# theislab/dca

Measured on AMD Instinct MI355X. Metric: cells/sec training (ZINB AE, 68k x 20k), higher is better.
Workload: dtype f32

## Files before the change

### dca_amd/csrc/dcahip_heads.hip

```cpp
#include <hip/hip_runtime.h>
#include <stdint.h>
#include <type_traits>
#include "dcahip.h"
#include "zinb_math.hpp"

namespace {

using f32x16 = __attribute__((ext_vector_type(16))) float;

constexpr int kTG = 32;
constexpr int kTR = 32;
constexpr int kLdS = 33;
constexpr int kWG = 2;
constexpr int kMaxGrid = 2048;
constexpr int kMaxSmallGrid = 8192;
constexpr int kCUs = 256;
constexpr int kZU = 4;
constexpr int kQCap = 320;

__device__ __forceinline__ int rowmap(int e, int hi) { return (e & 3) + 8 * (e >> 2) + 4 * hi; }

__device__ __forceinline__ void wave_sync() {
    __builtin_amdgcn_fence(__ATOMIC_RELEASE, "wavefront");
    __builtin_amdgcn_wave_barrier();
// ... 43 lines not shown
        f[0][j] = a; f[1][j] = b;
    }
}
#ifdef DCA_EXP_H2_TWO
#define MFMA_H3(A, Bf, ACC) { ACC = MFMAH(A[0], Bf[1], ACC); ACC = MFMAH(A[0], Bf[0], ACC); }
#else
#define MFMA_H3(A, Bf, ACC) { ACC = MFMAH(A[1], Bf[0], ACC); ACC = MFMAH(A[0], Bf[1], ACC); ACC = MFMAH(A[0], Bf[0], ACC); }
#endif

__device__ __forceinline__ float pow2i(int e) { return __uint_as_float((unsigned)(127 + e) << 23); }
__device__ __forceinline__ int block_exp(float m) {
    if (!(m > 0.f) || !(m < INFINITY)) return 0;
    const int e = kTop + 1 - __builtin_amdgcn_frexp_expf(m);
    return e < -60 ? -60 : (e > 60 ? 60 : e);
}
__device__ __forceinline__ float wave_max(float v) {
    int l = (int)__builtin_amdgcn_mbcnt_hi(~0u, __builtin_amdgcn_mbcnt_lo(~0u, 0u));
    asm volatile("" : "+v"(l));
#pragma unroll
    for (int off = 32; off > 0; off >>= 1)
        v = fmaxf(v, __int_as_float(__builtin_amdgcn_ds_bpermute((l ^ off) << 2, __float_as_int(v))));
    return v;
}

struct HeadsArgs2 {
    const unsigned short* HA;
    const unsigned short* HT;
    const int* eH;
    const float* H; long ldh;
    float* gW; long ldg;
    float* g_theta;
    const float* Wh; long ldw;
    const float* bh;
    const float* theta_w;
    const float* y;  long ldy;
    const unsigned char* yc; long ldc;
    const int* ovf_ptr; const int* ovf_col; const float* ovf_val;
    const float* sf;
    const int* perm;
    const long long* cursor;
    float* ws_dw;  long dw_stride;
    float* ws_dh;
    int npart, nitems;
    const int* tile_order;
    double* partials;
    long plane, ldws;
    int B, hL, G;
    int S, NT;
    float ridge, inv_n;
    int d_exp;
    int tile_base;
};

__device__ __forceinline__ float escaped_count(const HeadsArgs2& p, long srow, int col) {
    float v = 255.f;
    if (p.ovf_ptr)
        for (int i = p.ovf_ptr[srow], e = p.ovf_ptr[srow + 1]; i < e; ++i)
            if (p.ovf_col[i] == col) { v = p.ovf_val[i]; break; }
    return v;
}

__global__ __launch_bounds__(256) void heads_split_h_kernel(const float* H, long ldh, int B, int hL,
                                                            unsigned short* HA, unsigned short* HT, int* eH) {
    __shared__ unsigned short tr[2][64][32 + 2];
    __shared__ float wm[4];
    const int t = blockIdx.x, tid = threadIdx.x;
    const int row = tid >> 3, k0 = (tid & 7) * 8;
    const long grow = (long)t * 32 + row;
    float x[8];
    float m = 0.f;
#pragma unroll
    for (int j = 0; j < 8; ++j) {
        x[j] = (grow < B && k0 + j < hL) ? H[grow * ldh + k0 + j] : 0.f;
        m = fmaxf(m, fabsf(x[j]));
    }
    m = wave_max(m);
    if ((tid & 63) == 0) wm[tid >> 6] = m;
    __syncthreads();
    const int e = block_exp(fmaxf(fmaxf(wm[0], wm[1]), fmaxf(wm[2], wm[3])));
    if (tid == 0) eH[t] = (fmaxf(fmaxf(wm[0], wm[1]), fmaxf(wm[2], wm[3])) > 0.f) ? e : kEHZero;
    const float sc = pow2i(e);
#pragma unroll
    for (int j = 0; j < 8; ++j) x[j] *= sc;
    u32x4 f[2];
    split8(x, f);
    const int pos = (row & 0x13) | ((row & 4) << 1) | ((row & 8) >> 1);
#pragma unroll
    for (int q = 0; q < 2; ++q) {
        *reinterpret_cast<u32x4*>(HA + (((long)t * 2 + q) * 32 + row) * 64 + k0) = f[q];
#pragma unroll
        for (int j = 0; j < 8; ++j) tr[q][k0 + j][pos] = (unsigned short)(f[q][j >> 1] >> (16 * (j & 1)));
    }
    __syncthreads();
    for (int c = tid; c < 2 * 64 * 4; c += 256) {
        const int q = c >> 8, i = (c >> 2) & 63, part = c & 3;
        u32x4 v;
#pragma unroll
        for (int j = 0; j < 4; ++j) v[j] = (unsigned)tr[q][i][part * 8 + 2 * j] | ((unsigned)tr[q][i][part * 8 + 2 * j + 1] << 16);
        *reinterpret_cast<u32x4*>(HT + (((long)t * 2 + q) * 64 + i) * 32 + part * 8) = v;
    }
}

template <bool HAS_PI, bool CONST_DISP, bool YC>
__global__ __launch_bounds__(64 * kWR2) void heads_fused_h2_kernel(HeadsArgs2 p) {
    using YV = std::conditional_t<YC, unsigned, float>;
    constexpr int WR = kWR2;
    constexpr int NH = 1 + (CONST_DISP ? 0 : 1) + (HAS_PI ? 1 : 0);
    constexpr int PI_H = NH - 1;
    constexpr int KT = 64;
    constexpr int ST_PLANE = kTG * kLdS;
    constexpr int QCAP = 192;
    constexpr int CELL_LD = 144;
    constexpr int HEAD_B = kTG * CELL_LD;
    constexpr int ROWT = 96;
    constexpr int PW_FLOATS = NH * HEAD_B / 4 + (CONST_DISP ? ST_PLANE : 0) + QCAP * 4 + ROWT;
    constexpr int NTHREADS = 64 * WR;
    constexpr int W_PIECE = 64 * 64;
    constexpr int W_FLOATS = NH * 2 * W_PIECE / 4;
    constexpr int NRED = NH * 2 * 16 + NH + 1;
    constexpr int BIAS_FLOATS = (NH + 1) * 32;
    constexpr int LDS_FLOATS = W_FLOATS + WR * PW_FLOATS + BIAS_FLOATS;
    static_assert((WR / 2) * NRED * 64 <= LDS_FLOATS, "dW reduce scratch");
    __shared__ __attribute__((aligned(16))) float lds[LDS_FLOATS];
    __shared__ double lred[WR];
    __shared__ float wmaxs[WR];

    const int tid = threadIdx.x, lane = tid & 63;
    const int wave = __builtin_amdgcn_readfirstlane(tid >> 6);
    const int l31 = lane & 31, hi = lane >> 5;
    const int r = wave;
    const long long cur = p.cursor ? *p.cursor : 0;
    double dacc = 0.0;
    bool first_item = true;
    const int s_wg = blockIdx.x % p.S, wq = blockIdx.x / p.S;
    const int ngb = p.nitems / p.S;
    const int full = ngb / p.npart, rem = ngb - full * p.npart;
    const int nrounds = full + ((rem > 0 && ((full & 1) ? p.npart - 1 - wq : wq) < rem) ? 1 : 0);
    const int kD0 = kDExp0 + p.d_exp;
    int eHmin = 1 << 20;
    for (int t = s_wg * WR + r; t < p.NT; t += p.S * WR) { const int e = p.eH[t]; eHmin = (e != kEHZero && e < eHmin) ? e : eHmin; }
    eHmin = __builtin_amdgcn_readfirstlane(eHmin == (1 << 20) ? 0 : eHmin);
    int srow_l = 0;
    float sf_l = 1.f;
    int eHt = 0;
    u32x4 ha0[2] = {};
    bool carried = false;
#pragma unroll 1
    for (int j = 0; j < nrounds; ++j) {
    const int gb = j * p.npart + ((j & 1) ? p.npart - 1 - wq : wq);
    int s_opaque = s_wg;
    asm volatile("" : "+v"(s_opaque));
    const int s = __builtin_amdgcn_readfirstlane(s_opaque);
    const int gt = p.tile_order ? p.tile_order[gb + p.tile_base] : gb + p.tile_base;
    const int g0 = gt * kTG;
    const int gene = g0 + l31;
    const bool tile_ok = g0 < p.G;
    const bool gvalid = gene < p.G;

    unsigned char* const Wimg = reinterpret_cast<unsigned char*>(lds);
    unsigned char* const Pimg = reinterpret_cast<unsigned char*>(lds + W_FLOATS + wave * PW_FLOATS);
    float* const Th = lds + W_FLOATS + wave * PW_FLOATS + NH * HEAD_B / 4;
    u32x4* const Qe = reinterpret_cast<u32x4*>(lds + W_FLOATS + wave * PW_FLOATS + NH * HEAD_B / 4 + (CONST_DISP ? ST_PLANE : 0));
    float* const Bs = lds + W_FLOATS + WR * PW_FLOATS;
    int* const Rt = reinterpret_cast<int*>(lds + W_FLOATS + wave * PW_FLOATS + PW_FLOATS - ROWT);
    float* const Sft = reinterpret_cast<float*>(Rt + 64);

    const int gene_c = gvalid ? gene : p.G - 1;
    const float* const ycol = p.y + gene_c;
    const unsigned char* const ycolc = p.yc + gene_c;
    const unsigned ldy_u = YC ? (unsigned)p.ldc : (unsigned)p.ldy;
    auto count_at = [&](int sr) -> YV {
        if constexpr (YC) return (unsigned)ycolc[(unsigned long long)(unsigned)sr * ldy_u];
        else return ycol[(unsigned long long)(unsigned)sr * ldy_u];
    };
    YV yA[kZU], yB[kZU];
    auto row_clamped = [&](int tt) { const int rl = tt * kTR + l31; return rl < p.B ? rl : p.B - 1; };
    auto load_srow = [&](int tt) { const int rlc = row_clamped(tt); return p.perm ? p.perm[cur + rlc] : (int)(cur + rlc); };
    const __amdgpu_buffer_rsrc_t ha_rs = __builtin_amdgcn_make_buffer_rsrc(
        const_cast<unsigned short*>(p.HA), 0, p.NT * (kHTile * 2), 0x00020000);
    const int ha_lane = l31 * 128 + hi * 64;
    auto load_ha = [&](int tt, int ks, u32x4 (&dst)[2]) {
        const int so = tt * (kHTile * 2);
        int ha_o = ha_lane;
        asm volatile("" : "+v"(ha_o));
#pragma unroll
        for (int q = 0; q < 2; ++q)
            dst[q] = __builtin_bit_cast(u32x4, __builtin_amdgcn_raw_buffer_load_b128(ha_rs, ha_o + q * 4096 + ks * 16, so, 0));
    };
    const int t0 = s * WR + r;
    if (tile_ok && t0 < p.NT && !carried) {
        srow_l = load_srow(t0);
        eHt = p.eH[t0];
        sf_l = p.sf[srow_l];
        load_ha(t0, 0, ha0);
    }
    auto item_head = [&]() {
        if (lane < 32) Rt[l31] = srow_l;
        wave_sync();
        const int4 r4 = *reinterpret_cast<const int4*>(Rt + 4 * hi);
        yA[0] = count_at(r4.x); yA[1] = count_at(r4.y); yA[2] = count_at(r4.z); yA[3] = count_at(r4.w);
    };

    int eW = 0;
    if (tile_ok) {
        constexpr int UNR = (NH * 64 * 8 + NTHREADS - 1) / NTHREADS;
        constexpr int ITEMS = NH * 64 * 8;
        float4 v[UNR];
        int tidp = tid;
        asm volatile("" : "+v"(tidp));
        float m = 0.f;
#pragma unroll
        for (int u = 0; u < UNR; ++u) {
            const int idx = tidp + u * NTHREADS;
            const int c4 = idx & 7, kq = (idx >> 3) & 63, h = (idx >> 9) < NH ? (idx >> 9) : NH - 1;
            const int kc = kq < p.hL ? kq : p.hL - 1;
            long gcol = g0 + c4 * 4;
            if (gcol > p.plane - 4) gcol = p.plane - 4;
            v[u] = *reinterpret_cast<const float4*>(p.Wh + (long)kc * p.ldw + (long)h * p.plane + gcol);
        }
        float bv[NH + 1];
#pragma unroll
        for (int h = 0; h < NH; ++h) bv[h] = p.bh[(long)h * p.plane + gene_c];
        bv[NH] = CONST_DISP ? p.theta_w[gene_c] : 0.f;
        item_head();
#pragma unroll
        for (int u = 0; u < UNR; ++u) {
            const int idx = tidp + u * NTHREADS;
            const int c4 = idx & 7, kq = (idx >> 3) & 63;
            const int gcol = g0 + c4 * 4;
            const bool kv = idx < ITEMS && kq < p.hL && gcol <= p.plane - 4;
            if (!kv || gcol + 0 >= p.G) v[u].x = 0.f;
            if (!kv || gcol + 1 >= p.G) v[u].y = 0.f;
            if (!kv || gcol + 2 >= p.G) v[u].z = 0.f;
            if (!kv || gcol + 3 >= p.G) v[u].w = 0.f;
            m = fmaxf(fmaxf(m, fmaxf(fabsf(v[u].x), fabsf(v[u].y))), fmaxf(fabsf(v[u].z), fabsf(v[u].w)));
        }
        m = wave_max(m);
        if (lane == 0) wmaxs[wave] = m;
        __syncthreads();
        m = fmaxf(fmaxf(fmaxf(wmaxs[0], wmaxs[1]), fmaxf(wmaxs[2], wmaxs[3])), fmaxf(fmaxf(wmaxs[4], wmaxs[5]), fmaxf(wmaxs[6], wmaxs[7])));
        eW = __builtin_amdgcn_readfirstlane(block_exp(m));
        const float wsc = pow2i(eW);
#pragma unroll
        for (int u = 0; u < UNR; ++u) {
            const int idx = tidp + u * NTHREADS;
            if (idx >= ITEMS) continue;
            const int c4 = idx & 7, kq = (idx >> 3) & 63, h = idx >> 9;
            unsigned a0, a1, b0, b1;
            split_pair(v[u].x * wsc, v[u].y * wsc, a0, a1);
            split_pair(v[u].z * wsc, v[u].w * wsc, b0, b1);
            const int off = kq * 64 + ((((c4 >> 1) + (kq >> 2)) & 3) << 4) + ((c4 & 1) << 3);
            *reinterpret_cast<u32x2*>(Wimg + (h * 2 + 0) * W_PIECE + off) = u32x2{a0, b0};
            *reinterpret_cast<u32x2*>(Wimg + (h * 2 + 1) * W_PIECE + off) = u32x2{a1, b1};
        }
        if (tid < 32) {
#pragma unroll
            for (int h = 0; h < NH; ++h) Bs[h * 32 + tid] = gvalid ? bv[h] : 0.f;
            Bs[NH * 32 + tid] = (CONST_DISP && gvalid) ? bv[NH] : 0.f;
        }
    }
    __syncthreads();

    f32x16 dW[NH][2];
#pragma unroll
    for (int h = 0; h < NH; ++h)
#pragma unroll
        for (int ib = 0; ib < 2; ++ib)
#pragma unroll
            for (int e = 0; e < 16; ++e) dW[h][ib][e] = 0.f;
    float bsum[NH];
#pragma unroll
    for (int h = 0; h < NH; ++h) bsum[h] = 0.f;
    float thsum = 0.f;

    if (tile_ok) {
        const int tstep = p.S * WR;
        int t = t0;
        const long dh_tstride = (long)p.npart * (kTR * KT);
        float* const dh_part = p.ws_dh + (long)(blockIdx.x / p.S) * (kTR * KT);
        const int dh_lane = ((((l31 & 0x13) | ((l31 & 4) << 1) | ((l31 & 8) >> 1)) * KT) + 4 * hi) * 4;
        const __amdgpu_buffer_rsrc_t ht_rs = __builtin_amdgcn_make_buffer_rsrc(
            const_cast<unsigned short*>(p.HT), 0, p.NT * (kHTile * 2), 0x00020000);
        const int ht_lane = l31 * 64 + hi * 16;
        auto load_ht = [&](int tt, int ks, u32x4 (&dst)[2][2]) {
            const int so = tt * (kHTile * 2);
            int ht_o = ht_lane;
            asm volatile("" : "+v"(ht_o));
#pragma unroll
            for (int q = 0; q < 2; ++q)
#pragma unroll
                for (int ib = 0; ib < 2; ++ib)
                    dst[q][ib] = __builtin_bit_cast(u32x4, __builtin_amdgcn_raw_buffer_load_b128(
                        ht_rs, ht_o + q * 4096 + ib * 2048 + ks * 32, so, 0));
        };
// ... 346 lines not shown
                            u32x4 bf[2] = {w_dr(h, 0, jb, gs), w_dr(h, 1, jb, gs)};
                            MFMA_H3(bf, af, dHa[jb])
                        }
                    }
#pragma unroll
                for (int jb = 0; jb < 2; ++jb)
#pragma unroll
                    for (int eq = 0; eq < 4; ++eq) {
                        u32x4 v;
#pragma unroll
                        for (int w = 0; w < 4; ++w) v[w] = __float_as_uint(dHa[jb][4 * eq + w] * fu);
                        __builtin_amdgcn_raw_buffer_store_b128(v, dh_rs, dh_o + 128 * jb + 32 * eq, 0, 0);
                    }
            }
            srow_l = srow_n;
            sf_l = sf_n;
            eHt = eHn;
            if (lane < 32) Sft[l31] = sf_n;
            rb ^= 1;
            wave_sync();
        }
        carried = carried || t0 < p.NT;
        {
#pragma unroll
            for (int h = 0; h < NH; ++h)
#pragma unroll
                for (int ib = 0; ib < 2; ++ib)
#pragma unroll
                    for (int e = 0; e < 16; ++e) dW[h][ib][e] = __builtin_amdgcn_ldexpf(dW[h][ib][e], -accE);
        }
    }

    __syncthreads();

    {
        float* red = lds;
#pragma unroll
        for (int step = 1; step < WR; step *= 2) {
            const int slot = r / (2 * step);
            float* rs = red + (long)slot * NRED * 64 + lane;
            if (r % (2 * step) == step) {
                int n = 0;
#pragma unroll
                for (int h = 0; h < NH; ++h)
#pragma unroll
                    for (int ib = 0; ib < 2; ++ib)
#pragma unroll
                        for (int e = 0; e < 16; ++e) rs[(n++) * 64] = dW[h][ib][e];
#pragma unroll
                for (int h = 0; h < NH; ++h) rs[(n++) * 64] = bsum[h];
                rs[(n++) * 64] = thsum;
            }
            __syncthreads();
            if (r % (2 * step) == 0 && r + step < WR) {
                int n = 0;
#pragma unroll
                for (int h = 0; h < NH; ++h)
#pragma unroll
                    for (int ib = 0; ib < 2; ++ib)
#pragma unroll
                        for (int e = 0; e < 16; ++e) dW[h][ib][e] += rs[(n++) * 64];
#pragma unroll
                for (int h = 0; h < NH; ++h) bsum[h] += rs[(n++) * 64];
                thsum += rs[(n++) * 64];
            }
            __syncthreads();
        }
    }
    if (r == 0 && tile_ok) {
        const bool direct = p.S == 1;
        float* out = direct ? p.gW : p.ws_dw + (long)s * p.dw_stride;
        const long ldo = direct ? p.ldg : p.ldws;
        const float fin = direct ? p.inv_n : 1.f;
        const bool cw = gene < p.plane;
#pragma unroll
        for (int h = 0; h < NH; ++h) {
#pragma unroll
            for (int ib = 0; ib < 2; ++ib)
#pragma unroll
                for (int e = 0; e < 16; ++e) {
                    const int i = ib * 32 + rowmap(e, hi);
                    if (cw && i < p.hL) out[(long)i * ldo + (long)h * p.plane + gene] = dW[h][ib][e] * fin;
                }
            const float bv = bsum[h] + __shfl_xor(bsum[h], 32, 64);
            if (cw && hi == 0) out[(long)p.hL * ldo + (long)h * p.plane + gene] = bv * fin;
        }
        if (CONST_DISP) {
            const float tv = thsum + __shfl_xor(thsum, 32, 64);
            if (direct) {
                if (gvalid && hi == 0) {
                    const float e = expf(p.theta_w[gene]);
                    p.g_theta[gene] = (e >= 1e-3f && e <= 1e4f) ? tv * p.inv_n * e : 0.f;
                }
            } else if (cw && hi == 0) {
                out[(long)(p.hL + 1) * ldo + gene] = tv;
            }
        }
    }
    __syncthreads();
    first_item = false;
    }
// ... 131 lines not shown
    if (loss_out && bid == 0) {
        __shared__ double lsum[256];
        double a = 0.0;
        for (int i = threadIdx.x; i < n_partials; i += 256) a += loss_partials[i];
        lsum[threadIdx.x] = a;
        __syncthreads();
        for (int st = 128; st > 0; st >>= 1) {
            if ((int)threadIdx.x < st) lsum[threadIdx.x] += lsum[threadIdx.x + st];
            __syncthreads();
        }
        if (threadIdx.x == 0) {
            float lf = (float)(lsum[0] * loss_scale);
            if (isnan(lf)) lf = INFINITY;
            *loss_out = lf;
        }
    }
}

template <int GL>
__global__ __launch_bounds__(256) void heads_reduce_dh_kernel(ReduceDhArgs q) { reduce_dh_body<GL>(q, blockIdx.x); }

template <int GL>
__global__ __launch_bounds__(256) void heads_reduce_both_kernel(ReduceDhArgs qh, ReduceDwArgs qw, int n_dh) {
    if ((int)blockIdx.x < n_dh) reduce_dh_body<GL>(qh, blockIdx.x);
    else reduce_dw_body(qw, blockIdx.x - n_dh, gridDim.x - n_dh);
}


struct HeadsPlan {
    bool small;
    int HLB, WR, S, NT, ntg, ngb, grid;
    int nitems, npart;
    long ldws, dw_stride, dw_bytes, dh_bytes, hs_bytes;
    int nmain, ntail, S2, grid2, npart2, nitems2;
    long dh2_bytes, dw2_bytes;
};

inline bool al16(const void* p) { return (reinterpret_cast<uintptr_t>(p) & 15) == 0; }

bool make_heads_plan(int B, int hL, int G, long plane, int flags, HeadsPlan* out) {
    if (flags & (DCAHIP_NLL_POISSON | DCAHIP_NLL_MSE)) return false;
    if (B <= 0 || G <= 0 || hL <= 0 || hL > 64 || plane < G || (plane & 3) || plane > ((G + 31) & ~31)) return false;
    if (B > (1 << 22)) return false;
    const bool has_pi = flags & DCAHIP_NLL_HAS_PI, cdisp = flags & DCAHIP_NLL_CONST_DISP;
    const int NH = 1 + (cdisp ? 0 : 1) + (has_pi ? 1 : 0);
    HeadsPlan p;
    p.HLB = 2;
    p.NT = (B + kTR - 1) / kTR;
    p.ntg = (G + kTG - 1) / kTG;
    p.ngb = p.ntg;
    if (p.ngb > kMaxGrid) return false;
    p.small = p.NT < kWr8MinNT;
    static_assert((kWr8MinNT - 1) * kMaxGrid <= kMaxSmallGrid, "loss partials of the four-wave kernel");
    p.WR = p.small ? 1 : kWR2;
    const int smax = (p.NT + p.WR - 1) / p.WR;
    double best = 1e300;
    p.S = 1;
    const double item_cost = 0.75;
    for (int S = 1; S <= smax && (long)S * p.ngb <= kMaxGrid; ++S) {
        const long items = (long)S * p.ngb;
        const long rounds = (items + kCUs - 1) / kCUs;
        const int tiles = (p.NT + S * p.WR - 1) / (S * p.WR);
        const double cost = (double)rounds * (tiles + item_cost);
        if (cost < best - 1e-9) { best = cost; p.S = S; }
    }
    p.nitems = p.S * p.ngb;
// ... 10 lines not shown
        p.npart = p.grid / p.S;
    }
    p.nmain = p.ngb; p.ntail = 0; p.S2 = 0; p.grid2 = 0; p.npart2 = 0; p.nitems2 = 0;
    if (!p.small && p.S >= 2) {
        const int full = p.ngb / p.npart, rem = p.ngb - full * p.npart;
        const int tiles = (p.NT + p.S * p.WR - 1) / (p.S * p.WR);
        if (full >= 1 && rem > 0) {
            const double uniform = (double)(full + 1) * (tiles + item_cost);
            double best2 = 1e300; int bestS = 0;
            for (int S2 = 2 * p.S; S2 <= smax && (long)S2 * rem <= kMaxGrid; S2 *= 2) {
                const long items2 = (long)S2 * rem;
                const long rounds2 = (items2 + kCUs - 1) / kCUs;
                const int tiles2 = (p.NT + S2 * p.WR - 1) / (S2 * p.WR);
                const double c2 = (double)rounds2 * (tiles2 + item_cost);
                if (c2 < best2 - 1e-9) { best2 = c2; bestS = S2; }
            }
            if (bestS && (double)full * (tiles + item_cost) + best2 + 1.0 < uniform - 0.5) {
                p.nmain = full * p.npart; p.ntail = rem; p.S2 = bestS;
                p.nitems = p.S * p.nmain;
                p.nitems2 = p.S2 * p.ntail;
                const int res2 = kCUs / p.S2 * p.S2;
                p.grid2 = p.nitems2 < res2 ? p.nitems2 : res2;
                p.npart2 = p.grid2 / p.S2;
            }
        }
    }
    p.ldws = (long)NH * plane;
    p.dw_stride = (long)(hL + 2) * p.ldws;
    p.dw_bytes = (long)p.S * p.dw_stride * (long)sizeof(float);
    p.dh_bytes = (long)p.npart * p.NT * kTR * (p.HLB * 32) * (long)sizeof(float);
    p.dw2_bytes = (long)p.S2 * p.dw_stride * (long)sizeof(float);
    p.dh2_bytes = (long)p.npart2 * p.NT * kTR * (p.HLB * 32) * (long)sizeof(float);
    p.hs_bytes = 2L * p.NT * kHTile * 2 + (((long)p.NT * 4 + 15) & ~15L);
    *out = p;
    return true;
}

template <bool HAS_PI, bool CONST_DISP, bool YC>
__global__ __launch_bounds__(256) void heads_fused_small_kernel(HeadsArgs2 p) {
    using YV = std::conditional_t<YC, unsigned, float>;
    constexpr int NH = 1 + (CONST_DISP ? 0 : 1) + (HAS_PI ? 1 : 0);
    constexpr int PI_H = NH - 1;
    constexpr int KT = 64;
    constexpr int ST_PLANE = kTG * kLdS;
    constexpr int NP = NH + (CONST_DISP ? 1 : 0);
    constexpr int TH_P = NH;
    constexpr int ST_TILE = NP * ST_PLANE;
    constexpr int W_PIECE = 64 * 64;
    constexpr int W_FLOATS = NH * 2 * W_PIECE / 4;
    constexpr int BIAS_FLOATS = CONST_DISP ? (NH + 1) * 32 : 0;
    constexpr int NW = 4;
    static_assert(NW * kZU == 16, "one Z group per wave");
    constexpr int QCAP = kZU * 64;
    constexpr int LDS_FLOATS = W_FLOATS + ST_TILE + NW * QCAP + BIAS_FLOATS;
    static_assert(LDS_FLOATS * 4 + NW * 8 + 64 <= 42 * 1280, "three workgroups per CU (LDS is allocated in 1280-byte granules)");
    __shared__ __attribute__((aligned(16))) float lds[LDS_FLOATS];
    __shared__ double lred[NW];
    __shared__ float wmaxs[NW];
    __shared__ float dmaxs[NW];

    const int tid = threadIdx.x, lane = tid & 63;
    const int wave = __builtin_amdgcn_readfirstlane(tid >> 6);
    const int l31 = lane & 31, hi = lane >> 5;
    const long long cur = p.cursor ? *p.cursor : 0;
    const int t = p.NT > 1 ? (int)(blockIdx.x % p.NT) : 0;
    const int gb = p.NT > 1 ? (int)(blockIdx.x / p.NT) : (int)blockIdx.x;
// ... 383 lines not shown
    for (int k0 = 0; k0 < K; k0 += 16) {
        float av[8], bv[8];
#pragma unroll
        for (int j = 0; j < 8; ++j) {
            av[j] = A[(long)l31 * K + k0 + 8 * hi + j] * sa;
            bv[j] = B[(long)(k0 + 8 * hi + j) * 32 + l31] * sb;
        }
        u32x4 af[2], bf[2];
        split8(av, af);
        split8(bv, bf);
        MFMA_H3(af, bf, acc)
    }
    const float un = pow2i(-(ea + eb));
#pragma unroll
    for (int e = 0; e < 16; ++e) C[rowmap(e, hi) * 32 + l31] = acc[e] * un;
}

template <bool P, bool C, bool YC>
void launch_fused(const HeadsPlan& pl, const HeadsArgs2& a, hipStream_t s) {
    if (pl.small) hipLaunchKernelGGL((heads_fused_small_kernel<P, C, YC>), dim3(pl.grid), dim3(256), 0, s, a);
    else hipLaunchKernelGGL((heads_fused_h2_kernel<P, C, YC>), dim3(pl.grid), dim3(64 * kWR2), 0, s, a);
}

}

extern "C" long dcahip_heads_fused_workspace_bytes(int B, int hL, int G, long plane, int flags) {
    HeadsPlan p;
    if (!make_heads_plan(B, hL, G, plane, flags, &p)) return 0;
    long need = 0;
    for (int nt = 1; nt <= p.NT; ++nt) {
        const int b = nt * kTR < B ? nt * kTR : B;
        HeadsPlan q;
        if (!make_heads_plan(b, hL, G, plane, flags, &q)) continue;
        const long n = q.dw_bytes + q.dh_bytes + q.hs_bytes + q.dw2_bytes + q.dh2_bytes;
        if (n > need) need = n;
    }
    return need;
}

extern "C" int dcahip_x3_product_32x32(const float* A, const float* B, float* C, int K, void* stream) {
    if (!A || !B || !C || K <= 0 || (K & 15)) return DCAHIP_EINVAL;
    hipLaunchKernelGGL(x3_product_kernel, dim3(1), dim3(64), 0, static_cast<hipStream_t>(stream), A, B, C, K);
    return (int)hipGetLastError();
}

extern "C" int dcahip_heads_tile_order_len(int G) { return G > 0 ? (((G + kTG - 1) / kTG + kWG - 1) / kWG) * kWG : 0; }

extern "C" int dcahip_heads_fused(const float* H, long ldh, const float* Wh, long ldw,
                                  const float* bh, long plane, const float* theta_w,
                                  const float* y, long ldy,
                                  const unsigned char* yc, long ldc, const int* ovf_ptr, const int* ovf_col,
                                  const float* ovf_val, const float* sf, const int* perm,
                                  const long long* cursor, int B, int hL, int G, float ridge,
                                  float inv_n, int flags, float* gW, long ldg, float* g_theta,
                                  float* dH, long lddh, double* loss_partials, int* n_partials_out,
                                  void* workspace, long workspace_bytes, const int* tile_order,
                                  float* loss_out, int d_exp, void* stream) {
    const bool has_pi = flags & DCAHIP_NLL_HAS_PI, cdisp = flags & DCAHIP_NLL_CONST_DISP;
    HeadsPlan pl;
    if (!make_heads_plan(B, hL, G, plane, flags, &pl)) return DCAHIP_EINVAL;
    if (!H || !Wh || !bh || (!y && !yc) || !sf || !gW || !dH || !loss_partials || !workspace) return DCAHIP_EINVAL;
    if (cdisp && (!theta_w || !g_theta)) return DCAHIP_EINVAL;
    if (workspace_bytes < pl.dw_bytes + pl.dh_bytes + pl.hs_bytes + pl.dw2_bytes + pl.dh2_bytes) return DCAHIP_EINVAL;
    if (!al16(H) || !al16(Wh) || !al16(workspace) || (ldh & 3) || (ldw & 3) || ldh < ((hL + 3) & ~3))
        return DCAHIP_EINVAL;
    if (d_exp > 0 || d_exp < -24 || !(ridge >= 0.f) || ridge > 1e3f) return DCAHIP_EINVAL;
    const int NH = 1 + (cdisp ? 0 : 1) + (has_pi ? 1 : 0);
    if (ldw < (long)NH * plane || ldg < (long)NH * plane) return DCAHIP_EINVAL;
    if (yc ? (ldc < G || ldc > 0xffffffffL) : (ldy < G || ldy > 0xffffffffL)) return DCAHIP_EINVAL;
    float* ws_dh = static_cast<float*>(workspace);
    float* ws_dw = ws_dh + pl.dh_bytes / sizeof(float);
    float* ws_dh2 = ws_dw + pl.dw_bytes / sizeof(float);
    float* ws_dw2 = ws_dh2 + pl.dh2_bytes / sizeof(float);
    hipStream_t s = static_cast<hipStream_t>(stream);
    bool direct_dw = false;
    {
        unsigned short* HA = reinterpret_cast<unsigned short*>(reinterpret_cast<char*>(workspace) + pl.dh_bytes + pl.dw_bytes +
                                                               pl.dh2_bytes + pl.dw2_bytes);
        unsigned short* HT = HA + (long)pl.NT * kHTile;
        int* eH = reinterpret_cast<int*>(HT + (long)pl.NT * kHTile);
        if (!pl.small) {
            hipLaunchKernelGGL(heads_split_h_kernel, dim3(pl.NT), dim3(256), 0, s, H, ldh, B, hL, HA, HT, eH);
            int rc0 = (int)hipGetLastError();
            if (rc0 != 0) return rc0;
        }
        direct_dw = pl.S == 1;
        HeadsArgs2 a{HA, HT, eH, H, ldh, gW, ldg, g_theta, Wh, ldw, bh, theta_w, y, ldy, yc, ldc, ovf_ptr, ovf_col, ovf_val,
                     sf, perm, cursor, ws_dw, pl.dw_stride, ws_dh,
                     pl.npart, pl.nitems, tile_order, loss_partials, plane, pl.ldws, B, hL, G, pl.S, pl.NT, ridge, inv_n, d_exp, 0};
        auto launch = [&](const HeadsPlan& q, const HeadsArgs2& b) {
            if (yc) {
                if (has_pi && cdisp) launch_fused<true, true, true>(q, b, s);
                else if (has_pi) launch_fused<true, false, true>(q, b, s);
                else if (cdisp) launch_fused<false, true, true>(q, b, s);
                else launch_fused<false, false, true>(q, b, s);
            } else {
                if (has_pi && cdisp) launch_fused<true, true, false>(q, b, s);
                else if (has_pi) launch_fused<true, false, false>(q, b, s);
                else if (cdisp) launch_fused<false, true, false>(q, b, s);
                else launch_fused<false, false, false>(q, b, s);
            }
        };
        launch(pl, a);
        if (pl.ntail > 0) {
            HeadsPlan q2 = pl;
            q2.grid = pl.grid2; q2.S = pl.S2;
            HeadsArgs2 b = a;
            b.ws_dw = ws_dw2; b.ws_dh = ws_dh2; b.npart = pl.npart2; b.nitems = pl.nitems2; b.S = pl.S2;
            b.partials = loss_partials + pl.grid; b.tile_base = pl.nmain;
            launch(q2, b);
        }
    }
    int rc = (int)hipGetLastError();
    if (rc != 0) return rc;
    const int n_part = pl.grid + pl.grid2;
    if (n_partials_out) *n_partials_out = n_part;
    {
        const int KT = pl.HLB * 32;
        const long nq = (long)B * (KT / 4);
        const ReduceDhArgs qh{ws_dh, pl.npart, B, pl.NT * kTR, KT, hL, dH, lddh, inv_n, loss_partials, n_part, (double)inv_n, loss_out,
// ... 25 lines not shown
```

### include/dcahip.h

```cpp
#ifndef DCAHIP_H
#define DCAHIP_H

#ifdef __cplusplus
extern "C" {
#endif

#define DCAHIP_VERSION 2
#define DCAHIP_EINVAL (-22)

#define DCAHIP_NLL_HAS_PI      1
#define DCAHIP_NLL_CONST_DISP  2
#define DCAHIP_NLL_POISSON     4
#define DCAHIP_NLL_MSE         8

int dcahip_version(void);

int dcahip_zinb_max_partials(void);

int dcahip_zinb_nll(const float* a_mean, const float* a_disp, const float* a_pi, long lda,
                    const float* theta_w,
                    const float* y, long ldy, const float* sf,
                    const int* perm, const long long* cursor,
                    int B, int G, float ridge, float inv_n, int flags,
                    float* d_mean, float* d_disp, float* d_pi, long ldd,
// ... 20 lines not shown
                         double* cell_out, double* gene_acc, double* workspace, void* stream);

#define DCAHIP_GROUP_NO_SF   16
#define DCAHIP_GROUP_LOG1P   32
int dcahip_group_moments_workspace_doubles(int B, int G, int K);
int dcahip_group_moments(const float* a_mean, long lda, const float* sf, const int* codes,
                         int B, int G, int K, int flags,
                         double* sum_acc, double* sumsq_acc, long ldg,
                         double* workspace, void* stream);

long dcahip_ranksum_workspace_bytes(int g, int n);
int dcahip_ranksum(const float* x, long ldx, int g, int n,
                   const int* order, int m, const int* gstart, int K, int ref,
                   long long* rank2, long long* tie, long ldr,
                   void* workspace, void* stream);

long dcahip_gram_workspace_doubles(int B, int G);
int dcahip_gram(const float* x, long ldx, const int* cols, const int* keep, const double* shift,
                int B, int G, double* cross, long ldc, double* dsum, double* ws, void* stream);

int dcahip_loss_finalize(const double* partials, int n_partials, double scale,
                         float* loss_out, void* stream);

int dcahip_step_end(const float* loss, double weight, float* hist, int rows_per_slot,
                    double* acc, long long* cursor, int advance, void* stream);

int dcahip_zinb_heads_infer(const float* a_mean, const float* a_disp, const float* a_pi,
                            long lda, const float* sf, int B, int G,
                            float* mean_sf, float* theta, float* pi, long ldo, int flags,
                            void* stream);

long dcahip_heads_fused_workspace_bytes(int B, int hL, int G, long plane, int flags);
int dcahip_heads_tile_order_len(int G);
int dcahip_heads_fused(const float* H, long ldh, const float* Wh, long ldw, const float* bh,
                       long plane, const float* theta_w,
                       const float* y, long ldy,
                       const unsigned char* yc, long ldc, const int* ovf_ptr, const int* ovf_col,
                       const float* ovf_val, const float* sf,
                       const int* perm, const long long* cursor,
                       int B, int hL, int G, float ridge, float inv_n, int flags,
                       float* gW, long ldg, float* g_theta, float* dH, long lddh,
                       double* loss_partials, int* n_partials_out,
                       void* workspace, long workspace_bytes, const int* tile_order,
                       float* loss_out, int d_exp, void* stream);
int dcahip_x3_product_32x32(const float* A, const float* B, float* C, int K, void* stream);

int dcahip_sgemm(int ta, int tb, int M, int N, int K,
                 const float* A, long lda, const float* B, long ldb, float* C, long ldc,
                 const float* bias, const int* perm, const long long* cursor,
                 int colsum_row, int split_k, void* workspace, long workspace_bytes,
                 void* stream);
long dcahip_sgemm_workspace_bytes(int ta, int tb, int M, int N, int K, int colsum_row, int split_k);
int dcahip_sgemm_plan(int ta, int tb, int M, int N, int K, int colsum_row, int split_k,
                      const float* A, long lda, const float* B, long ldb, int out[8]);
int dcahip_split_planes(const float* src, long ld, const int* perm, const long long* cursor, long R, int C,
                        void* planes, long ldp, long plane_stride, void* stream);
int dcahip_gemm_p3(int ta, int tb, int M, int N, int K, const void* A, long lda, long plane_a,
                   const void* B, long ldb, long plane_b, float* C, long ldc, const float* bias,
                   const int* perm, const long long* cursor, int colsum_row, int split_k,
                   void* workspace, long workspace_bytes, void* stream);
long dcahip_gemm_p3_workspace_bytes(int M, int N, int K, int colsum_row, int split_k);
int dcahip_gemm_planes_plan(int pieces, int ta, int tb, int M, int N, int K, int gather, int colsum_row, int split_k, int out[12]);
int dcahip_absmax_exp(const float* src, long ld, long R, int C, int* exp_out, void* scratch_word, void* stream);
int dcahip_split_planes_h2(const float* src, long ld, const int* perm, const long long* cursor, long R, int C,
                           void* planes, long ldp, long plane_stride, const int* exp, void* stream);
int dcahip_gemm_h2_supported(int M, int N, int K);
// ... 233 lines not shown
```

Measured before the change: 4.367 million.

## Precompute split weight tile images in split kernel and prefetch next tile during reduce

Moves the per-tile weight split (scaling, bf16-style split into hi/lo pieces, bias/theta gather) out of the fused heads kernel into extra blocks of the H-split kernel, writing a per-tile record to workspace. The fused kernel then just loads the prebuilt record and issues the load for the next tile before the dW reduction, landing it into LDS after, overlapping global latency with reduction. The reduction scratch is shifted past the weight image to avoid clobbering it. It adds workspace memory and a global round-trip for the image.

```diff
diff --git a/dca_amd/csrc/dcahip_heads.hip b/dca_amd/csrc/dcahip_heads.hip
--- a/dca_amd/csrc/dcahip_heads.hip
+++ b/dca_amd/csrc/dcahip_heads.hip
@@ -99,6 +99,7 @@
     float* g_theta;
     const float* Wh; long ldw;
     const float* bh;
+    const unsigned char* wimg;
     const float* theta_w;
     const float* y;  long ldy;
     const unsigned char* yc; long ldc;
@@ -127,11 +128,11 @@
     return v;
 }
 
-__global__ __launch_bounds__(256) void heads_split_h_kernel(const float* H, long ldh, int B, int hL,
-                                                            unsigned short* HA, unsigned short* HT, int* eH) {
+__device__ __forceinline__ void split_h_body(const float* H, long ldh, int B, int hL,
+                                             unsigned short* HA, unsigned short* HT, int* eH, int t) {
     __shared__ unsigned short tr[2][64][32 + 2];
     __shared__ float wm[4];
-    const int t = blockIdx.x, tid = threadIdx.x;
+    const int tid = threadIdx.x;
     const int row = tid >> 3, k0 = (tid & 7) * 8;
     const long grow = (long)t * 32 + row;
     float x[8];
@@ -166,6 +167,79 @@
         for (int j = 0; j < 4; ++j) v[j] = (unsigned)tr[q][i][part * 8 + 2 * j] | ((unsigned)tr[q][i][part * 8 + 2 * j + 1] << 16);
         *reinterpret_cast<u32x4*>(HT + (((long)t * 2 + q) * 64 + i) * 32 + part * 8) = v;
     }
+}
+
+constexpr int kWPiece = 64 * 64;
+constexpr long wimg_rec_bytes(int NH) { return (long)NH * 2 * kWPiece + (NH + 1) * 32 * 4 + 16; }
+struct WImgArgs {
+    const float* Wh; long ldw; const float* bh; const float* theta_w;
+    long plane; int hL, G;
+    unsigned char* out;
+};
+
+template <int NH>
+__device__ __forceinline__ void wimage_body(const WImgArgs& q, int gt) {
+    __shared__ float wmaxs[4];
+    const int tid = threadIdx.x, lane = tid & 63, wave = tid >> 6;
+    const int g0 = gt * kTG;
+    unsigned char* const rec = q.out + (long)gt * wimg_rec_bytes(NH);
+    constexpr int UNR = 2 * NH;
+    float4 v[UNR];
+    float m = 0.f;
+#pragma unroll
+    for (int u = 0; u < UNR; ++u) {
+        const int idx = tid + u * 256;
+        const int c4 = idx & 7, kq = (idx >> 3) & 63, h = idx >> 9;
+        const int kc = kq < q.hL ? kq : q.hL - 1;
+        long gcol = g0 + c4 * 4;
+        if (gcol > q.plane - 4) gcol = q.plane - 4;
+        v[u] = *reinterpret_cast<const float4*>(q.Wh + (long)kc * q.ldw + (long)h * q.plane + gcol);
+    }
+#pragma unroll
+    for (int u = 0; u < UNR; ++u) {
+        const int idx = tid + u * 256;
+        const int c4 = idx & 7, kq = (idx >> 3) & 63;
+        const int gcol = g0 + c4 * 4;
+        const bool kv = kq < q.hL && gcol <= q.plane - 4;
+        if (!kv || gcol + 0 >= q.G) v[u].x = 0.f;
+        if (!kv || gcol + 1 >= q.G) v[u].y = 0.f;
+        if (!kv || gcol + 2 >= q.G) v[u].z = 0.f;
+        if (!kv || gcol + 3 >= q.G) v[u].w = 0.f;
+        m = fmaxf(fmaxf(m, fmaxf(fabsf(v[u].x), fabsf(v[u].y))), fmaxf(fabsf(v[u].z), fabsf(v[u].w)));
+    }
+    m = wave_max(m);
+    if (lane == 0) wmaxs[wave] = m;
+    __syncthreads();
+    const int eW = block_exp(fmaxf(fmaxf(wmaxs[0], wmaxs[1]), fmaxf(wmaxs[2], wmaxs[3])));
+    const float wsc = pow2i(eW);
+#pragma unroll
+    for (int u = 0; u < UNR; ++u) {
+        const int idx = tid + u * 256;
+        const int c4 = idx & 7, kq = (idx >> 3) & 63, h = idx >> 9;
+        unsigned a0, a1, b0, b1;
+        split_pair(v[u].x * wsc, v[u].y * wsc, a0, a1);
+        split_pair(v[u].z * wsc, v[u].w * wsc, b0, b1);
+        const int off = kq * 64 + ((((c4 >> 1) + (kq >> 2)) & 3) << 4) + ((c4 & 1) << 3);
+        *reinterpret_cast<u32x2*>(rec + (h * 2 + 0) * kWPiece + off) = u32x2{a0, b0};
+        *reinterpret_cast<u32x2*>(rec + (h * 2 + 1) * kWPiece + off) = u32x2{a1, b1};
+    }
+    float* const rows = reinterpret_cast<float*>(rec + NH * 2 * kWPiece);
+    if (tid < 32) {
+        const int gene = g0 + tid;
+        const bool gvalid = gene < q.G;
+#pragma unroll
+        for (int h = 0; h < NH; ++h) rows[h * 32 + tid] = gvalid ? q.bh[(long)h * q.plane + gene] : 0.f;
+        rows[NH * 32 + tid] = (q.theta_w && gvalid) ? q.theta_w[gene] : 0.f;
+    } else if (tid < 36) {
+        reinterpret_cast<int*>(rows + (NH + 1) * 32)[tid - 32] = tid == 32 ? eW : 0;
+    }
+}
+
+template <int NH>
+__global__ __launch_bounds__(256) void heads_split_kernel(const float* H, long ldh, int B, int hL, unsigned short* HA,
+                                                          unsigned short* HT, int* eH, int n_h, WImgArgs q) {
+    if ((int)blockIdx.x < n_h) split_h_body(H, ldh, B, hL, HA, HT, eH, blockIdx.x);
+    else wimage_body<NH>(q, blockIdx.x - n_h);
 }
 
 template <bool HAS_PI, bool CONST_DISP, bool YC>
@@ -182,15 +256,17 @@
     constexpr int ROWT = 96;
     constexpr int PW_FLOATS = NH * HEAD_B / 4 + (CONST_DISP ? ST_PLANE : 0) + QCAP * 4 + ROWT;
     constexpr int NTHREADS = 64 * WR;
-    constexpr int W_PIECE = 64 * 64;
+    constexpr int W_PIECE = kWPiece;
     constexpr int W_FLOATS = NH * 2 * W_PIECE / 4;
     constexpr int NRED = NH * 2 * 16 + NH + 1;
-    constexpr int BIAS_FLOATS = (NH + 1) * 32;
+    constexpr int BIAS_FLOATS = (NH + 1) * 32 + 4;
     constexpr int LDS_FLOATS = W_FLOATS + WR * PW_FLOATS + BIAS_FLOATS;
-    static_assert((WR / 2) * NRED * 64 <= LDS_FLOATS, "dW reduce scratch");
+    constexpr int IMG_B = NH * 2 * W_PIECE;
+    constexpr int NBQ = BIAS_FLOATS / 4;
+    static_assert(IMG_B == NH * NTHREADS * 16 && IMG_B + NBQ * 16 == wimg_rec_bytes(NH) && NBQ <= 64, "record layout");
+    static_assert((WR / 2) * NRED * 64 <= WR * PW_FLOATS, "dW reduce scratch");
     __shared__ __attribute__((aligned(16))) float lds[LDS_FLOATS];
     __shared__ double lred[WR];
-    __shared__ float wmaxs[WR];
 
     const int tid = threadIdx.x, lane = tid & 63;
     const int wave = __builtin_amdgcn_readfirstlane(tid >> 6);
@@ -212,35 +288,12 @@
     int eHt = 0;
     u32x4 ha0[2] = {};
     bool carried = false;
-#pragma unroll 1
-    for (int j = 0; j < nrounds; ++j) {
-    const int gb = j * p.npart + ((j & 1) ? p.npart - 1 - wq : wq);
-    int s_opaque = s_wg;
-    asm volatile("" : "+v"(s_opaque));
-    const int s = __builtin_amdgcn_readfirstlane(s_opaque);
-    const int gt = p.tile_order ? p.tile_order[gb + p.tile_base] : gb + p.tile_base;
-    const int g0 = gt * kTG;
-    const int gene = g0 + l31;
-    const bool tile_ok = g0 < p.G;
-    const bool gvalid = gene < p.G;
-
     unsigned char* const Wimg = reinterpret_cast<unsigned char*>(lds);
-    unsigned char* const Pimg = reinterpret_cast<unsigned char*>(lds + W_FLOATS + wave * PW_FLOATS);
-    float* const Th = lds + W_FLOATS + wave * PW_FLOATS + NH * HEAD_B / 4;
-    u32x4* const Qe = reinterpret_cast<u32x4*>(lds + W_FLOATS + wave * PW_FLOATS + NH * HEAD_B / 4 + (CONST_DISP ? ST_PLANE : 0));
     float* const Bs = lds + W_FLOATS + WR * PW_FLOATS;
     int* const Rt = reinterpret_cast<int*>(lds + W_FLOATS + wave * PW_FLOATS + PW_FLOATS - ROWT);
     float* const Sft = reinterpret_cast<float*>(Rt + 64);
-
-    const int gene_c = gvalid ? gene : p.G - 1;
-    const float* const ycol = p.y + gene_c;
-    const unsigned char* const ycolc = p.yc + gene_c;
     const unsigned ldy_u = YC ? (unsigned)p.ldc : (unsigned)p.ldy;
-    auto count_at = [&](int sr) -> YV {
-        if constexpr (YC) return (unsigned)ycolc[(unsigned long long)(unsigned)sr * ldy_u];
-        else return ycol[(unsigned long long)(unsigned)sr * ldy_u];
-    };
-    YV yA[kZU], yB[kZU];
+    YV yA[kZU];
     auto row_clamped = [&](int tt) { const int rl = tt * kTR + l31; return rl < p.B ? rl : p.B - 1; };
     auto load_srow = [&](int tt) { const int rlc = row_clamped(tt); return p.perm ? p.perm[cur + rlc] : (int)(cur + rlc); };
     const __amdgpu_buffer_rsrc_t ha_rs = __builtin_amdgcn_make_buffer_rsrc(
@@ -254,79 +307,80 @@
         for (int q = 0; q < 2; ++q)
             dst[q] = __builtin_bit_cast(u32x4, __builtin_amdgcn_raw_buffer_load_b128(ha_rs, ha_o + q * 4096 + ks * 16, so, 0));
     };
-    const int t0 = s * WR + r;
-    if (tile_ok && t0 < p.NT && !carried) {
-        srow_l = load_srow(t0);
-        eHt = p.eH[t0];
-        sf_l = p.sf[srow_l];
-        load_ha(t0, 0, ha0);
-    }
-    auto item_head = [&]() {
+    auto tile_at = [&](int jj) {
+        const int gbn = jj * p.npart + ((jj & 1) ? p.npart - 1 - wq : wq);
+        return __builtin_amdgcn_readfirstlane(p.tile_order ? p.tile_order[gbn + p.tile_base] : gbn + p.tile_base);
+    };
+    const int t0w = s_wg * WR + r;
+    u32x4 wv[NH], bq;
+    auto item_request = [&](int gtn) {
+        if (gtn * kTG >= p.G) return;
+        if (t0w < p.NT && !carried) {
+            srow_l = load_srow(t0w);
+            eHt = p.eH[t0w];
+            sf_l = p.sf[srow_l];
+            load_ha(t0w, 0, ha0);
+        }
+        int tidp = tid;
+        asm volatile("" : "+v"(tidp));
+        const unsigned char* const rec = p.wimg + (long)gtn * (IMG_B + NBQ * 16);
+#pragma unroll
+        for (int u = 0; u < NH; ++u) wv[u] = *reinterpret_cast<const u32x4*>(rec + (tidp + u * NTHREADS) * 16);
+        bq = *reinterpret_cast<const u32x4*>(rec + IMG_B + (tidp < NBQ ? tidp : NBQ - 1) * 16);
+    };
+    auto item_land = [&](int gtn) {
+        if (gtn * kTG >= p.G) return;
+        const int gn = gtn * kTG + l31;
+        const int gcn = gn < p.G ? gn : p.G - 1;
         if (lane < 32) Rt[l31] = srow_l;
         wave_sync();
         const int4 r4 = *reinterpret_cast<const int4*>(Rt + 4 * hi);
-        yA[0] = count_at(r4.x); yA[1] = count_at(r4.y); yA[2] = count_at(r4.z); yA[3] = count_at(r4.w);
-    };
-
-    int eW = 0;
-    if (tile_ok) {
-        constexpr int UNR = (NH * 64 * 8 + NTHREADS - 1) / NTHREADS;
-        constexpr int ITEMS = NH * 64 * 8;
-        float4 v[UNR];
+        const int rr[kZU] = {r4.x, r4.y, r4.z, r4.w};
+#pragma unroll
+        for (int i = 0; i < kZU; ++i) {
+            if constexpr (YC) yA[i] = (unsigned)(p.yc + gcn)[(unsigned long long)(unsigned)rr[i] * ldy_u];
+            else yA[i] = (p.y + gcn)[(unsigned long long)(unsigned)rr[i] * ldy_u];
+        }
         int tidp = tid;
         asm volatile("" : "+v"(tidp));
-        float m = 0.f;
-#pragma unroll
-        for (int u = 0; u < UNR; ++u) {
-            const int idx = tidp + u * NTHREADS;
-            const int c4 = idx & 7, kq = (idx >> 3) & 63, h = (idx >> 9) < NH ? (idx >> 9) : NH - 1;
-            const int kc = kq < p.hL ? kq : p.hL - 1;
-            long gcol = g0 + c4 * 4;
-            if (gcol > p.plane - 4) gcol = p.plane - 4;
-            v[u] = *reinterpret_cast<const float4*>(p.Wh + (long)kc * p.ldw + (long)h * p.plane + gcol);
-        }
-        float bv[NH + 1];
-#pragma unroll
-        for (int h = 0; h < NH; ++h) bv[h] = p.bh[(long)h * p.plane + gene_c];
-        bv[NH] = CONST_DISP ? p.theta_w[gene_c] : 0.f;
-        item_head();
-#pragma unroll
-        for (int u = 0; u < UNR; ++u) {
-            const int idx = tidp + u * NTHREADS;
-            const int c4 = idx & 7, kq = (idx >> 3) & 63;
-            const int gcol = g0 + c4 * 4;
-            const bool kv = idx < ITEMS && kq < p.hL && gcol <= p.plane - 4;
-            if (!kv || gcol + 0 >= p.G) v[u].x = 0.f;
-            if (!kv || gcol + 1 >= p.G) v[u].y = 0.f;
-            if (!kv || gcol + 2 >= p.G) v[u].z = 0.f;
-            if (!kv || gcol + 3 >= p.G) v[u].w = 0.f;
-            m = fmaxf(fmaxf(m, fmaxf(fabsf(v[u].x), fabsf(v[u].y))), fmaxf(fabsf(v[u].z), fabsf(v[u].w)));
-        }
-        m = wave_max(m);
-        if (lane == 0) wmaxs[wave] = m;
-        __syncthreads();
-        m = fmaxf(fmaxf(fmaxf(wmaxs[0], wmaxs[1]), fmaxf(wmaxs[2], wmaxs[3])), fmaxf(fmaxf(wmaxs[4], wmaxs[5]), fmaxf(wmaxs[6], wmaxs[7])));
-        eW = __builtin_amdgcn_readfirstlane(block_exp(m));
-        const float wsc = pow2i(eW);
-#pragma unroll
-        for (int u = 0; u < UNR; ++u) {
-            const int idx = tidp + u * NTHREADS;
-            if (idx >= ITEMS) continue;
-            const int c4 = idx & 7, kq = (idx >> 3) & 63, h = idx >> 9;
-            unsigned a0, a1, b0, b1;
-            split_pair(v[u].x * wsc, v[u].y * wsc, a0, a1);
-            split_pair(v[u].z * wsc, v[u].w * wsc, b0, b1);
-            const int off = kq * 64 + ((((c4 >> 1) + (kq >> 2)) & 3) << 4) + ((c4 & 1) << 3);
-            *reinterpret_cast<u32x2*>(Wimg + (h * 2 + 0) * W_PIECE + off) = u32x2{a0, b0};
-            *reinterpret_cast<u32x2*>(Wimg + (h * 2 + 1) * W_PIECE + off) = u32x2{a1, b1};
-        }
-        if (tid < 32) {
-#pragma unroll
-            for (int h = 0; h < NH; ++h) Bs[h * 32 + tid] = gvalid ? bv[h] : 0.f;
-            Bs[NH * 32 + tid] = (CONST_DISP && gvalid) ? bv[NH] : 0.f;
-        }
+#pragma unroll
+        for (int u = 0; u < NH; ++u) *reinterpret_cast<u32x4*>(Wimg + (tidp + u * NTHREADS) * 16) = wv[u];
+        if (tidp < NBQ) *reinterpret_cast<u32x4*>(reinterpret_cast<unsigned char*>(Bs) + tidp * 16) = bq;
+    };
+    int gt_next = 0;
+    if (nrounds > 0) {
+        gt_next = tile_at(0);
+        item_request(gt_next);
+        item_land(gt_next);
     }
     __syncthreads();
+#pragma unroll 1
+    for (int j = 0; j < nrounds; ++j) {
+    int s_opaque = s_wg;
+    asm volatile("" : "+v"(s_opaque));
+    const int s = __builtin_amdgcn_readfirstlane(s_opaque);
+    const int gt = gt_next;
+    const bool has_next = j + 1 < nrounds;
+    if (has_next) gt_next = tile_at(j + 1);
+    const int g0 = gt * kTG;
+    const int gene = g0 + l31;
+    const bool tile_ok = g0 < p.G;
+    const bool gvalid = gene < p.G;
+
+    unsigned char* const Pimg = reinterpret_cast<unsigned char*>(lds + W_FLOATS + wave * PW_FLOATS);
+    float* const Th = lds + W_FLOATS + wave * PW_FLOATS + NH * HEAD_B / 4;
+    u32x4* const Qe = reinterpret_cast<u32x4*>(lds + W_FLOATS + wave * PW_FLOATS + NH * HEAD_B / 4 + (CONST_DISP ? ST_PLANE : 0));
+
+    const int gene_c = gvalid ? gene : p.G - 1;
+    const float* const ycol = p.y + gene_c;
+    const unsigned char* const ycolc = p.yc + gene_c;
+    auto count_at = [&](int sr) -> YV {
+        if constexpr (YC) return (unsigned)ycolc[(unsigned long long)(unsigned)sr * ldy_u];
+        else return ycol[(unsigned long long)(unsigned)sr * ldy_u];
+    };
+    YV yB[kZU];
+    const int t0 = s * WR + r;
+    const int eW = tile_ok ? __builtin_amdgcn_readfirstlane(*reinterpret_cast<const int*>(Bs + (NH + 1) * 32)) : 0;
 
     f32x16 dW[NH][2];
 #pragma unroll
@@ -739,9 +793,10 @@
     }
 
     __syncthreads();
+    if (has_next) item_request(gt_next);
 
     {
-        float* red = lds;
+        float* red = lds + W_FLOATS;
 #pragma unroll
         for (int step = 1; step < WR; step *= 2) {
             const int slot = r / (2 * step);
@@ -774,6 +829,7 @@
             __syncthreads();
         }
     }
+    if (has_next) item_land(gt_next);
     if (r == 0 && tile_ok) {
         const bool direct = p.S == 1;
         float* out = direct ? p.gW : p.ws_dw + (long)s * p.dw_stride;
@@ -971,6 +1027,7 @@
     int HLB, WR, S, NT, ntg, ngb, grid;
     int nitems, npart;
     long ldws, dw_stride, dw_bytes, dh_bytes, hs_bytes;
+    long wi_bytes;
     int nmain, ntail, S2, grid2, npart2, nitems2;
     long dh2_bytes, dw2_bytes;
 };
@@ -1047,6 +1104,7 @@
     p.dw2_bytes = (long)p.S2 * p.dw_stride * (long)sizeof(float);
     p.dh2_bytes = (long)p.npart2 * p.NT * kTR * (p.HLB * 32) * (long)sizeof(float);
     p.hs_bytes = 2L * p.NT * kHTile * 2 + (((long)p.NT * 4 + 15) & ~15L);
+    p.wi_bytes = p.small ? 0 : (long)p.ntg * wimg_rec_bytes(NH);
     *out = p;
     return true;
 }
@@ -1496,10 +1554,16 @@
         const int b = nt * kTR < B ? nt * kTR : B;
         HeadsPlan q;
         if (!make_heads_plan(b, hL, G, plane, flags, &q)) continue;
-        const long n = q.dw_bytes + q.dh_bytes + q.hs_bytes + q.dw2_bytes + q.dh2_bytes;
+        const long n = q.dw_bytes + q.dh_bytes + q.hs_bytes + q.dw2_bytes + q.dh2_bytes + q.wi_bytes;
         if (n > need) need = n;
     }
     return need;
+}
+
+extern "C" long dcahip_heads_fused_wimage_offset(int B, int hL, int G, long plane, int flags) {
+    HeadsPlan p;
+    if (!make_heads_plan(B, hL, G, plane, flags, &p) || p.small) return -1;
+    return p.dh_bytes + p.dw_bytes + p.dh2_bytes + p.dw2_bytes + p.hs_bytes;
 }
 
 extern "C" int dcahip_x3_product_32x32(const float* A, const float* B, float* C, int K, void* stream) {
@@ -1525,7 +1589,7 @@
     if (!make_heads_plan(B, hL, G, plane, flags, &pl)) return DCAHIP_EINVAL;
     if (!H || !Wh || !bh || (!y && !yc) || !sf || !gW || !dH || !loss_partials || !workspace) return DCAHIP_EINVAL;
     if (cdisp && (!theta_w || !g_theta)) return DCAHIP_EINVAL;
-    if (workspace_bytes < pl.dw_bytes + pl.dh_bytes + pl.hs_bytes + pl.dw2_bytes + pl.dh2_bytes) return DCAHIP_EINVAL;
+    if (workspace_bytes < pl.dw_bytes + pl.dh_bytes + pl.hs_bytes + pl.dw2_bytes + pl.dh2_bytes + pl.wi_bytes) return DCAHIP_EINVAL;
     if (!al16(H) || !al16(Wh) || !al16(workspace) || (ldh & 3) || (ldw & 3) || ldh < ((hL + 3) & ~3))
         return DCAHIP_EINVAL;
     if (d_exp > 0 || d_exp < -24 || !(ridge >= 0.f) || ridge > 1e3f) return DCAHIP_EINVAL;
@@ -1543,13 +1607,18 @@
                                                                pl.dh2_bytes + pl.dw2_bytes);
         unsigned short* HT = HA + (long)pl.NT * kHTile;
         int* eH = reinterpret_cast<int*>(HT + (long)pl.NT * kHTile);
+        unsigned char* wimg = reinterpret_cast<unsigned char*>(HA) + pl.hs_bytes;
         if (!pl.small) {
-            hipLaunchKernelGGL(heads_split_h_kernel, dim3(pl.NT), dim3(256), 0, s, H, ldh, B, hL, HA, HT, eH);
+            const WImgArgs qi{Wh, ldw, bh, cdisp ? theta_w : nullptr, plane, hL, G, wimg};
+            const dim3 grid(pl.NT + pl.ntg);
+            if (NH == 3) hipLaunchKernelGGL(heads_split_kernel<3>, grid, dim3(256), 0, s, H, ldh, B, hL, HA, HT, eH, pl.NT, qi);
+            else if (NH == 2) hipLaunchKernelGGL(heads_split_kernel<2>, grid, dim3(256), 0, s, H, ldh, B, hL, HA, HT, eH, pl.NT, qi);
+            else hipLaunchKernelGGL(heads_split_kernel<1>, grid, dim3(256), 0, s, H, ldh, B, hL, HA, HT, eH, pl.NT, qi);
             int rc0 = (int)hipGetLastError();
             if (rc0 != 0) return rc0;
         }
         direct_dw = pl.S == 1;
-        HeadsArgs2 a{HA, HT, eH, H, ldh, gW, ldg, g_theta, Wh, ldw, bh, theta_w, y, ldy, yc, ldc, ovf_ptr, ovf_col, ovf_val,
+        HeadsArgs2 a{HA, HT, eH, H, ldh, gW, ldg, g_theta, Wh, ldw, bh, wimg, theta_w, y, ldy, yc, ldc, ovf_ptr, ovf_col, ovf_val,
                      sf, perm, cursor, ws_dw, pl.dw_stride, ws_dh,
                      pl.npart, pl.nitems, tile_order, loss_partials, plane, pl.ldws, B, hL, G, pl.S, pl.NT, ridge, inv_n, d_exp, 0};
         auto launch = [&](const HeadsPlan& q, const HeadsArgs2& b) {
diff --git a/include/dcahip.h b/include/dcahip.h
--- a/include/dcahip.h
+++ b/include/dcahip.h
@@ -76,6 +76,7 @@
 
 long dcahip_heads_fused_workspace_bytes(int B, int hL, int G, long plane, int flags);
 int dcahip_heads_tile_order_len(int G);
+long dcahip_heads_fused_wimage_offset(int B, int hL, int G, long plane, int flags);
 int dcahip_heads_fused(const float* H, long ldh, const float* Wh, long ldw, const float* bh,
                        long plane, const float* theta_w,
                        const float* y, long ldy,
```

New measurement: 4.365 million. Within noise of the previous version (-0.0%).
